# sipposip/pr-disagg-radar-gan

Hardware: AMD Instinct MI355X
Metric: cWGAN-GP train samples/sec, 24x16x16 tiles, bs=256 (higher is better)
Workload: dtype f32; 1 GPU; ndomain=16, 24h, bs=256 fp32, 1 critic step + 1 gen step (BASELINE configs[1]); batch_per_gpu=256, global_batch=256, n_critic=1, parallelism=dp1, world=1, rccl_ranks_seen=1, weights=random init (RandomNormal 0.02 / glorot_uniform), dropout 0.25 active

## Files before the change

### include/rdgan.h

```cpp
#ifndef RDGAN_H
#define RDGAN_H
#include <stdint.h>
#ifdef __cplusplus
extern "C" {
#endif

typedef struct rdgan_handle rdgan_handle;

#define RDGAN_LATENT_DIM 100
#define RDGAN_NHOURS 24
#define RDGAN_LOSS_SLOTS 8

int rdgan_create(rdgan_handle** out, int ndomain, int n_cond_channels, int max_batch);
void rdgan_destroy(rdgan_handle* h);
const char* rdgan_last_error(const rdgan_handle* h);
long rdgan_gen_param_count(const rdgan_handle* h);
long rdgan_critic_param_count(const rdgan_handle* h);
long rdgan_workspace_bytes(const rdgan_handle* h);

int rdgan_gen_forward(rdgan_handle* h, const float* gen_params, const float* z, const float* cond,
                      float* out, int B, void* stream);

int rdgan_check_numerics(rdgan_handle* h, void* stream);

// ... 132 lines not shown
                               int Cin, int Cout, int Do, int Ho, int Wo, int stride, int pad_d, int pad_h,
                               int pad_w, void* stream);
int rdgan_op_fastd_wgrad(const float* src, const float* dy, float* dU, int B, int D, int H, int W, int Cin, int Cout,
                         int g, int bf16, void* stream);
int rdgan_op_g9_wgrad(const float* dl, const float* h3, float* dW, int B, int nd, int bf16, int kernel, void* stream);
int rdgan_op_upconv_slab16(const float* x, const float* w, const float* bias, float* y, float* rinv, float* dbg, int B, void* stream);
int rdgan_op_upconv_slab_t16(const float* x, const float* w, const float* bias, float* y, float* rinv, float* dbg, int B, int H, int W,
                             void* stream);
int rdgan_op_upconv2_slab16(const float* x, const float* w, const float* bias, float* y, float* rinv, int B, void* stream);
int rdgan_op_upconv_wgrad_slab16(const float* x, const float* dy, float* dWc, int B, void* stream);
int rdgan_op_d2_fwd_slab16(const float* x, const float* w, const float* bias, float* y, int B, uint64_t seed, void* stream);
int rdgan_op_d2_wgrad_slab16(const float* x, const float* dy, float* dW, int B, void* stream);
int rdgan_op_d2_wgrad_slab_t16(const float* x, const float* dy, float* dW, int B, int OH, int OW, void* stream);
int rdgan_op_d3_wgrad_slab16(const float* x, const float* dy, float* dW, int B, void* stream);
int rdgan_op_d2_dgrad_slab16(const float* gy, const float* w, const float* aux, float* gx, int B, int use_drop, void* stream);
int rdgan_op_d2_dgrad_slab_t16(const float* gy, const float* w, const float* aux, float* gx, int B, int OH, int OW, int use_drop,
                               void* stream);
int rdgan_op_pixelnorm_lrelu(const float* y, float* h, float* rinv, long npix, int C, void* stream);
int rdgan_op_pixelnorm_lrelu_bwd(const float* gh, const float* h, const float* rinv, float* dy,
                                 long npix, int C, void* stream);
int rdgan_debug_activation(rdgan_handle* h, int which, float* out, long n, void* stream);
int rdgan_debug_d1_input_grad(rdgan_handle* h, const float* critic_params, const float* u1, int B, int with_norm,
                              float* g0_out, float* cin_hat_out, float* gp_out, void* stream);
int rdgan_op_rng(uint64_t seed, uint32_t stream_id, float* mask_out, float* uniform_out, long n,
                 void* stream);

#ifdef __cplusplus
}
#endif
#endif
```

### pr_disagg_radar_gan_amd/_lib.py

```python
import ctypes
import os

_HERE = os.path.dirname(os.path.abspath(__file__))
LIB_PATH = os.path.join(_HERE, "librdgan_hip.so")

c_f32p = ctypes.c_void_p
c_stream = ctypes.c_void_p

class LaunchStat(ctypes.Structure):
    _fields_ = [("plan", ctypes.c_int), ("kind", ctypes.c_int), ("batch", ctypes.c_int), ("launches", ctypes.c_int),
                ("gflop", ctypes.c_double), ("ms", ctypes.c_double), ("name", ctypes.c_char * 48), ("kernel", ctypes.c_char * 48)]


SIGNATURES = {
    "rdgan_create": (ctypes.c_int, [ctypes.POINTER(ctypes.c_void_p), ctypes.c_int, ctypes.c_int, ctypes.c_int]),
    "rdgan_destroy": (None, [ctypes.c_void_p]),
    "rdgan_last_error": (ctypes.c_char_p, [ctypes.c_void_p]),
    "rdgan_gen_param_count": (ctypes.c_long, [ctypes.c_void_p]),
    "rdgan_critic_param_count": (ctypes.c_long, [ctypes.c_void_p]),
    "rdgan_workspace_bytes": (ctypes.c_long, [ctypes.c_void_p]),
    "rdgan_gen_forward": (ctypes.c_int, [ctypes.c_void_p, c_f32p, c_f32p, c_f32p, c_f32p, ctypes.c_int, c_stream]),
    "rdgan_check_numerics": (ctypes.c_int, [ctypes.c_void_p, c_stream]),
    "rdgan_critic_forward": (ctypes.c_int, [ctypes.c_void_p, c_f32p, c_f32p, c_f32p, c_f32p, ctypes.c_int,
                                            ctypes.c_uint64, c_stream]),
# ... 73 lines not shown
    "rdgan_op_conv3d": (ctypes.c_int, [c_f32p, c_f32p, c_f32p, c_f32p] + [ctypes.c_int] * 14 + [c_stream]),
    "rdgan_op_conv3d_bf16": (ctypes.c_int, [c_f32p, c_f32p, c_f32p, c_f32p] + [ctypes.c_int] * 14 + [c_stream]),
    "rdgan_op_conv3d_dgrad": (ctypes.c_int, [c_f32p, c_f32p, c_f32p] + [ctypes.c_int] * 13 + [c_stream]),
    "rdgan_op_conv3d_wgrad_bf16": (ctypes.c_int, [c_f32p, c_f32p, c_f32p] + [ctypes.c_int] * 13 + [c_stream]),
    "rdgan_op_conv3d_dgrad_bf16": (ctypes.c_int, [c_f32p, c_f32p, c_f32p] + [ctypes.c_int] * 13 + [c_stream]),
    "rdgan_op_conv3d_wgrad": (ctypes.c_int, [c_f32p, c_f32p, c_f32p] + [ctypes.c_int] * 14 + [c_stream]),
    "rdgan_op_fastd_wgrad": (ctypes.c_int, [c_f32p, c_f32p, c_f32p] + [ctypes.c_int] * 8 + [c_stream]),
    "rdgan_op_g9_wgrad": (ctypes.c_int, [c_f32p, c_f32p, c_f32p] + [ctypes.c_int] * 4 + [c_stream]),
    "rdgan_op_upconv_slab16": (ctypes.c_int, [c_f32p] * 6 + [ctypes.c_int, c_stream]),
    "rdgan_op_upconv_slab_t16": (ctypes.c_int, [c_f32p] * 6 + [ctypes.c_int] * 3 + [c_stream]),
    "rdgan_op_upconv2_slab16": (ctypes.c_int, [c_f32p] * 5 + [ctypes.c_int, c_stream]),
    "rdgan_op_upconv_wgrad_slab16": (ctypes.c_int, [c_f32p] * 3 + [ctypes.c_int, c_stream]),
    "rdgan_op_d2_fwd_slab16": (ctypes.c_int, [c_f32p] * 4 + [ctypes.c_int, ctypes.c_uint64, c_stream]),
    "rdgan_op_d3_wgrad_slab16": (ctypes.c_int, [c_f32p] * 3 + [ctypes.c_int, c_stream]),
    "rdgan_op_d2_wgrad_slab16": (ctypes.c_int, [c_f32p] * 3 + [ctypes.c_int, c_stream]),
    "rdgan_op_d2_wgrad_slab_t16": (ctypes.c_int, [c_f32p] * 3 + [ctypes.c_int] * 3 + [c_stream]),
    "rdgan_op_d2_dgrad_slab16": (ctypes.c_int, [c_f32p] * 4 + [ctypes.c_int, ctypes.c_int, c_stream]),
    "rdgan_op_d2_dgrad_slab_t16": (ctypes.c_int, [c_f32p] * 4 + [ctypes.c_int] * 4 + [c_stream]),
    "rdgan_op_pixelnorm_lrelu": (ctypes.c_int, [c_f32p, c_f32p, c_f32p, ctypes.c_long, ctypes.c_int, c_stream]),
    "rdgan_op_pixelnorm_lrelu_bwd": (ctypes.c_int, [c_f32p, c_f32p, c_f32p, c_f32p, ctypes.c_long, ctypes.c_int, c_stream]),
    "rdgan_debug_activation": (ctypes.c_int, [ctypes.c_void_p, ctypes.c_int, c_f32p, ctypes.c_long, c_stream]),
    "rdgan_debug_d1_input_grad": (ctypes.c_int, [ctypes.c_void_p, c_f32p, c_f32p, ctypes.c_int, ctypes.c_int, c_f32p, c_f32p, c_f32p,
                                                 c_stream]),
    "rdgan_op_rng": (ctypes.c_int, [ctypes.c_uint64, ctypes.c_uint32, c_f32p, c_f32p, ctypes.c_long, c_stream]),
}

TAG_GCONV_FWD, TAG_GCONV_DGRAD, TAG_GCONV_WGRAD, TAG_CRITIC_GEMM, TAG_ELEMENTWISE, TAG_GCONV3_FWD = range(6)

_lib = None


class RdganError(RuntimeError):
    pass


class NumericsError(RdganError, ArithmeticError):
    """tf.debugging.check_numerics behind the generator's softmax (reference T:349-350) fired: NaN/Inf in the output."""


def load():
    global _lib
    if _lib is not None:
        return _lib
    if not os.path.exists(LIB_PATH):
        raise RdganError(
            f"{LIB_PATH} is missing: build it with `python -m pr_disagg_radar_gan_amd.build` "
# ... 19 lines not shown
```

### pr_disagg_radar_gan_amd/csrc/rdgan_api.hip

```cpp
#include <hip/hip_runtime.h>
#include <stdio.h>
#include <string.h>
#include <math.h>
#include <string>
#include <vector>
#include <algorithm>
#include <unordered_set>

#include "../../include/rdgan.h"
#include "rdgan_plan.h"
#include "rdgan_hostplan.h"
#include "rdgan_rng.h"
#include "rdgan_gemm.hip.h"
#include "rdgan_gemm_ws.hip.h"
#include "rdgan_gemm_ws16.hip.h"
#include "rdgan_gemm_f16.hip.h"
#include "rdgan_upconv16.hip.h"
#include "rdgan_upconv16b.hip.h"
#include "rdgan_upconv16t.hip.h"
#include "rdgan_elem.hip.h"
#include "rdgan_data.hip.h"
#include "rdgan_edge.hip.h"
#include "rdgan_d2slab16.hip.h"
#include "rdgan_d2fwd16.hip.h"
#include "rdgan_upwgrad16.hip.h"
#include "rdgan_upwgrad16b.hip.h"
#include "rdgan_d2wgrad16.hip.h"
#include "rdgan_d3wgrad16.hip.h"
#include "rdgan_d1fwd16.hip.h"
#include "rdgan_g9bwd16.hip.h"
#include "rdgan_spectral.hip.h"
#include "rdgan_rainfarm.hip.h"
#include "rdgan_crps.hip.h"
#include "rdgan_dist.hip.h"
#include "rdgan_radar.hip.h"
#include "rdgan_field.hip.h"
#include "rdgan_products.hip.h"
static_assert(RDGAN_LOSS_SLOTS == 8, "k_critic_losses / k_gen_loss write slots 0..7");
static bool g9w_mfma_ok(int nd, long npix) { return nd >= 8 && nd <= 128 && (nd & (nd - 1)) == 0 && npix < 0x7FFFFFFFL; }
static size_t g9w_mfma_lds(bool bf16) { return std::max<size_t>((size_t)128 * (bf16 ? 128 : 256) + (1440 + 144) * sizeof(float), 32768); }

#define RD_GP_WEIGHT 10.0f



struct RdLaunchRec { int plan, kind, batch; double flops; char kernel[48]; hipEvent_t e0, e1; };

struct rdgan_handle : RdGeom {
  std::string err;
  std::vector<RdPlan> plans;
  RdPlan* d_plans = nullptr;
  RdRow* d_tab = nullptr;
  char* ws = nullptr;
  size_t ws_bytes = 0;
  float *xcat, *h0, *h1, *r1, *h2, *r2, *h3, *r3, *P9, *fake, *dl, *gh3, *gup3, *dy2, *gup2, *dy1, *gup1, *ga0;
  float *cin, *dh[5], *du[5], *v, *P1, *g0, *gpv;
  float* ubias_part = nullptr;
  float *wpartial, *cpartial, *kpartial;
  size_t wpartial_cap = 0, cpartial_cap = 0, kpartial_cap = 0;
  float *DWT[5], *W1T, *GWT[4], *W9T, *W1P, *dW1P;
  float *fE[4], *fU[4], *fgS, *fdE, *fdU, *fUT;
  void *bU[4], *bUT;
  void *bWF[5], *bWB[5];
  void *bG1F[4], *bG1B, *bW1B;
  void *fWF[5], *fWB[5], *fG1F[4], *fG1B;
  int wgrad_wide = 0;
  int conv_f16 = 1;
  void* bW3I;
// ... 26 lines not shown
  int d2_slab = 1;
  int a16 = 0;
  int g9_direct = 1;
  int fast_fwd = -1;
  int fast_bwd = -1;
  float *GWC[4], *GWD[4], *dWc;
  int collapse = 1;
  int tapgather = 1;
  int ws_ksplit = 1;
  int wave_spec = 1;
  int resident = 1;
  int edge_kernels = 1;
  int sample_offset = 0;
  float* g9b_tmp;
  float* gp_part;
  float* dw6_part;
  int side_on = 1;
  int split3 = 0;
  int dense_slices = 0;
  uint64_t gver_in = 0, cver_in = 0;
  const float* gcache_ptr = nullptr; uint64_t gcache_ver = 0; int gcache_cfg = -1;
  const float* ccache_ptr = nullptr; uint64_t ccache_ver = 0; int ccache_cfg = -1;
  long form_builds[2] = {0, 0};
  int keep_gates = 0;
  void* gate_keep[5] = {nullptr, nullptr, nullptr, nullptr, nullptr};
  int gate_keep_B = 0;
  hipStream_t side = nullptr;
  hipEvent_t ev_fork = nullptr, ev_join = nullptr, ev_cw = nullptr, ev_g[4] = {nullptr, nullptr, nullptr, nullptr};
  int* d_flag;
  int fwd_ahead = -1;
  hipStream_t ahead = nullptr;
  hipEvent_t ev_ahead_fork = nullptr, ev_ahead_done = nullptr;
  float* kpartial_ahead = nullptr;
  int* flag_ahead = nullptr;
  bool ahead_pending = false;
  const float *ahead_gp = nullptr, *ahead_z = nullptr, *ahead_cond = nullptr;
  int ahead_B = 0;
  uint64_t ahead_gver = 0;
  std::unordered_set<const void*> lds_attr_done;
  int prof_launches = 0;
  std::vector<RdLaunchRec> launch_recs;
  size_t launch_used = 0;
  char cur_kernel[48] = {0};
  double flops_acc = 0;
  unsigned prof_mask = 0;
  std::vector<hipEvent_t> ev_start[RDGAN_NUM_TAGS], ev_stop[RDGAN_NUM_TAGS];
// ... 741 lines not shown
          carve(p, 27L * dch[l - 1] * dch[l] / 2 + 8); h->bWF[l] = p;
          carve(p, 27L * dch[l - 1] * dch[l] / 2 + 8); h->bWB[l] = p;
        }
        h->bG1F[0] = nullptr;
        for (int l = 1; l <= 3; ++l) { carve(p, 32L * gch[l - 1] * gch[l] + 8); h->bG1F[l] = p; }
        carve(p, 32L * 256 * 256 + 8); h->bG1B = p;
        h->fWF[0] = h->fWF[1] = h->fWB[0] = h->fWB[1] = h->fG1F[0] = nullptr;
        for (int l = 2; l <= 4; ++l) {
          carve(p, 27L * dch[l - 1] * dch[l] / 2 + 8); h->fWF[l] = p;
          carve(p, 27L * dch[l - 1] * dch[l] / 2 + 8); h->fWB[l] = p;
        }
        for (int l = 1; l <= 3; ++l) { carve(p, 32L * gch[l - 1] * gch[l] + 8); h->fG1F[l] = p; }
        carve(p, 32L * 256 * 256 + 8); h->fG1B = p;
        carve(p, 32L * h->ldp1 + 8); h->bW1B = p;
        carve(p, 64L * 8 * 2 * 64 * 4 + 8); h->bW3I = p;
        carve(p, 64L * 8 * 2 * 64 * 4 + 8); h->bW3T = p;
        carve(p, 4L * 64 * 4 + 8); h->bW9I = p;
        carve(p, (long)RD_UP2_KSTEPS * 4 * 64 * 4 + 8); h->bW2I = p;
        carve(p, (long)RD_D2S_KSTEPS * 2 * 64 * 4 + 8); h->bW2S = p;
        if (nd % 16 == 0) { carve(p, NB * h->dL[1] * 4 + 8); if (pass == 1) h->g1bits = (unsigned char*)p; }
        carve(p, (long)RD_D2F_KSTEPS * 4 * 64 * 4 + 8); h->bW2F = p;
      }
      carve(h->fdU, 48L * 256 * 256); carve(h->fUT, 48L * 256 * 256);
    }
    { float* f = nullptr; carve(f, 64); if (pass == 1) { h->d_flag = (int*)f; h->flag_ahead = (int*)f + 32; } }
    carve(h->g9b_tmp, 64);
    carve(h->ubias_part, 32 * 8 * 64);
    carve(h->gp_part, (size_t)MB * 64);
    carve(h->dw6_part, (size_t)16 * h->F);
    if (pass == 0) {
      h->ws_bytes = off + 256;
      e = hipMalloc((void**)&h->ws, h->ws_bytes);
      if (e != hipSuccess) { (void)hipFree(h->d_plans); delete h; return (int)e; }
      (void)hipMemset(h->ws, 0, h->ws_bytes);
    }
  }
  {
    bool ok = hipStreamCreateWithFlags(&h->side, hipStreamNonBlocking) == hipSuccess;
    hipEvent_t* evs[] = {&h->ev_fork, &h->ev_join, &h->ev_cw, &h->ev_g[1], &h->ev_g[2], &h->ev_g[3]};
    for (hipEvent_t* e2 : evs) ok = ok && hipEventCreateWithFlags(e2, hipEventDisableTiming) == hipSuccess;
    if (!ok) { h->side_on = 0; (void)hipGetLastError(); }
    bool ok2 = hipStreamCreateWithFlags(&h->ahead, hipStreamNonBlocking) == hipSuccess;
    ok2 = ok2 && hipEventCreateWithFlags(&h->ev_ahead_fork, hipEventDisableTiming) == hipSuccess;
    ok2 = ok2 && hipEventCreateWithFlags(&h->ev_ahead_done, hipEventDisableTiming) == hipSuccess;
    if (!ok2) { h->ahead = nullptr; (void)hipGetLastError(); }
  }
// ... 45 lines not shown
    if (value && !a16_geometry_ok(h->nd)) return bad_arg(h, RD_A16_TOO_LARGE);
    h->a16 = value ? 1 : 0; return 0;
  }
  if (!strcmp(name, "g9_direct")) { h->g9_direct = value ? 1 : 0; return 0; }
  if (!strcmp(name, "fast_fwd")) { h->fast_fwd = value < 0 ? -1 : (value ? 1 : 0); return 0; }
  if (!strcmp(name, "fast_bwd")) { h->fast_bwd = value < 0 ? -1 : (value ? 1 : 0); return 0; }
  if (!strcmp(name, "tapgather")) { h->tapgather = value ? 1 : 0; return 0; }
  if (!strcmp(name, "resident")) { h->resident = value ? 1 : 0; return 0; }
  if (!strcmp(name, "upconv_slab")) { h->upconv_slab = value ? 1 : 0; return 0; }
  if (!strcmp(name, "upconv_slab_t")) { h->upconv_slab_t = value ? 1 : 0; return 0; }
  if (!strcmp(name, "upconv2_slab")) { h->upconv2_slab = value ? 1 : 0; return 0; }
  if (!strcmp(name, "g9_fused")) { h->g9_fused = value ? 1 : 0; return 0; }
  if (!strcmp(name, "d1_fwd_sample")) { h->d1_fwd_sample = value ? 1 : 0; return 0; }
  if (!strcmp(name, "g9_bwd_mfma")) { h->g9_bwd_mfma = value ? 1 : 0; return 0; }
  if (!strcmp(name, "dense16")) { h->dense16 = value ? 1 : 0; return 0; }
  if (!strcmp(name, "dense_skinny")) { h->dense_skinny = value ? 1 : 0; return 0; }
  if (!strcmp(name, "wgrad_boxes")) { h->wgrad_boxes = value ? 1 : 0; return 0; }
  if (!strcmp(name, "border_boxes")) { h->border_boxes = value < 0 ? 0 : (value > 2 ? 2 : value); return 0; }
  if (!strcmp(name, "d3_wgrad_slab")) { h->d3_wgrad_slab = value ? 1 : 0; return 0; }
  if (!strcmp(name, "d2_wgrad_slab")) { h->d2_wgrad_slab = value ? 1 : 0; return 0; }
  if (!strcmp(name, "upwgrad_slab")) { h->upwgrad_slab = value ? 1 : 0; return 0; }
  if (!strcmp(name, "d1_dgrad_fused")) { h->d1_dgrad_fused = value ? 1 : 0; return 0; }
  if (!strcmp(name, "combine_dx_fused")) { h->combine_dx_fused = value ? 1 : 0; return 0; }
  if (!strcmp(name, "d1_wgrad16")) { h->d1_wgrad16 = value ? 1 : 0; return 0; }
  if (!strcmp(name, "wgrad_wide")) { h->wgrad_wide = value ? 1 : 0; return 0; }
  if (!strcmp(name, "conv_f16")) {
    if (value < 0 || value > 2) return bad_arg(h, "conv_f16: 0, 1 or 2 (2: regardless of the launch size)");
    h->conv_f16 = value; h->ccache_ver = 0; h->gcache_ver = 0; return 0;
  }
  if (!strcmp(name, "d2_fwd_slab")) { h->d2_fwd_slab = value ? 1 : 0; h->ccache_ver = 0; return 0; }
  if (!strcmp(name, "d2_gate_bits")) { h->d2_gate_bits = value ? 1 : 0; return 0; }
  if (!strcmp(name, "d2_slab")) { h->d2_slab = value ? 1 : 0; h->ccache_ver = 0; return 0; }
  if (!strcmp(name, "dense_wgrad_slices")) { h->dense_slices = value; return 0; }
  if (!strcmp(name, "keep_gates")) {
    h->keep_gates = value ? 1 : 0;
    h->gate_keep_B = 0;
    for (int l = 1; l <= 4 && h->keep_gates; ++l)
      if (!h->gate_keep[l]) RD_CHECK(h, hipMalloc(&h->gate_keep[l], (size_t)h->MB * h->dL[l] * h->dch[l] * sizeof(float)));
    return 0;
  }
  if (!strcmp(name, "split3")) { h->split3 = value ? 1 : 0; return 0; }
  if (!strcmp(name, "side_stream")) { h->side_on = (value && h->side) ? 1 : 0; return 0; }
  if (!strcmp(name, "gen_fwd_ahead")) { h->fwd_ahead = value < 0 ? -1 : (value ? 1 : 0); return 0; }
  if (!strcmp(name, "edge_kernels")) { h->edge_kernels = value < 0 ? 0 : (value > 2 ? 2 : value); return 0; }
  if (!strcmp(name, "sample_offset")) { if (value < 0) return bad_arg(h, "set_option: sample_offset < 0"); h->sample_offset = value; return 0; }
  if (!strcmp(name, "ws_ksplit")) { h->ws_ksplit = value < 0 ? 0 : (value > 8 ? 8 : value); return 0; }
// ... 157 lines not shown
static int critic_dgrad_plan(const rdgan_handle* h, int l, int n) {
  return critic_box_plan(h, PL_D2B + l - 2, PL_D2BX + l - 2, (long)n * h->dL[l - 1]);
}

static bool box_span_ok(const RdPlan& p, int B) {
  long minL = p.ph[0].L;
  for (int i = 1; i < p.nphases; ++i) minL = std::min<long>(minL, p.ph[i].L);
  return std::min<long>(B, 256 / minL + 2) * std::max(p.src_sample, p.dst_sample) * 4 < 0x7FFFFFF0L;
}
static int gen_box_plan(const rdgan_handle* h, int one, int box, int B) {
  if (!h->border_boxes || !h->plans[box].boxes || !box_span_ok(h->plans[box], B)) return one;
  if (h->border_boxes >= 2) return box;
  if (plan_flops(h->plans[box], 1) > 0.7 * plan_flops(h->plans[one], 1)) return one;
  return plan_tiles(h->plans[one], B, 128) * (h->plans[one].N / 128 > 0 ? h->plans[one].N / 128 : 1) >= 1024 ? box : one;
}

static int dense_skinny_ks(const rdgan_handle* h) { return (h->n_in + 127) / 128 * 8; }
static bool dense_skinny_on(const rdgan_handle* h) {
  return h->a16 && h->dense16 && h->dense_skinny && h->MB <= 128 && h->bW0 && h->xcat16 && h->n_nodes % 32 == 0 && h->KP0 % 64 == 0;
}
static bool g9_fused_on(const rdgan_handle* h) { return h->g9_fused && h->tapgather && upconv_slab_on(h, 3); }
static bool g9_fused_t_on(const rdgan_handle* h) { return h->g9_fused && h->tapgather && upconv_slab_t_on(h, 3); }

static int gen_forward_impl(rdgan_handle* h, const float* gp, const float* z, const float* cond, float* out, int B,
                            hipStream_t st, hipStream_t ws, bool keep_h3 = true) {
  const int nd = h->nd;
  const bool a16 = h->a16 != 0;
  RD_TRY(a16_check(h));
  const int gcfg = (h->collapse ? 1 : 0) | (fast_fwd_on(h) ? 2 : 0) | (a16 ? 4 : 0) | (h->upconv_slab ? 8 : 0) | (h->upconv2_slab ? 16 : 0) |
                   (h->g9_fused && h->tapgather ? 32 : 0) | (h->dense16 ? 64 : 0) | (h->upconv_slab_t ? 128 : 0) | (h->dense_skinny ? 256 : 0);
  const bool forms_cached = h->gver_in != 0 && gp == h->gcache_ptr && h->gver_in == h->gcache_ver && gcfg == h->gcache_cfg;
  if (!forms_cached) {
  h->form_builds[0]++;
  h->gcache_ptr = nullptr; h->gcache_ver = 0; h->gcache_cfg = -1;
  RD_TRY(launch_transpose(h, gp + h->goff[8], h->W9T, 1, 27, 64, 32, ws));
  if (dense_skinny_on(h)) {
    const long nimg = (long)(h->n_nodes / 32) * dense_skinny_ks(h) * 16;
    hipLaunchKernelGGL(k_dense_wimg, dim3((unsigned)((nimg + 255) / 256)), dim3(256), 0, ws, gp + h->goff[0], (unsigned short*)h->bW0,
                       h->n_in, h->n_nodes, dense_skinny_ks(h));
  } else
  if (a16 && h->dense16 && h->dense16_ok && h->bW0)
    hipLaunchKernelGGL(k_dense_w16, dim3((h->n_nodes + 31) / 32, (h->KP0 + 31) / 32), dim3(256), 0, ws, gp + h->goff[0],
                       (unsigned short*)h->bW0, h->n_in, h->n_nodes, h->KP0);
  if (g9_fused_on(h) || g9_fused_t_on(h)) hipLaunchKernelGGL(k_g9_wimg, dim3(1), dim3(256), 0, ws, gp + h->goff[8], (unsigned short*)h->bW9I);
  for (int l = 1; l <= 3; ++l) {
    const float* Wl = gp + h->goff[2 * l];
    const long cc = (long)h->gch[l - 1] * h->gch[l];
    if (gen_block_fast(h, l, fast_fwd_on(h))) {
      RdWeightMap wm;
      fastd_weight_map(wm);
      ProfScope ps(h, RDGAN_TAG_ELEMENTWISE, ws);
      hipLaunchKernelGGL(k_weight_transform, dim3(ew_blocks(48L * cc / 4)), dim3(256), 0, ws, Wl, h->fU[l], (int)cc, 48, wm);
      if (a16) RD_TRY(launch_weights_to_bf16_t(h, h->fU[l], h->bU[l], 48, h->gch[l - 1], h->gch[l], ws));
    } else if (h->collapse) {
      hipLaunchKernelGGL(k_collapse_weights, dim3(ew_blocks(16L * cc)), dim3(256), 0, ws, Wl, h->GWC[l], (int)cc);
      if (upconv_slab_on(h, l)) launch_upconv_wimg(h->GWC[l], h->bW3I, ws);
      else if (upconv_slab_t_on(h, l)) launch_upconv_wimg_t(h->GWC[l], h->bW3T, ws);
      else if (upconv2_slab_on(h, l)) launch_upconv2_wimg(h->GWC[l], h->bW2I, ws);
      else if (a16) {
        RD_TRY(launch_weights_to_bf16_t(h, h->GWC[l], h->bG1F[l], 64, h->gch[l - 1], h->gch[l], ws, h->conv_f16 ? h->fG1F[l] : nullptr));
      }
    }
    if (ws != st) RD_CHECK(h, hipEventRecord(h->ev_g[l], ws));
  }
  RD_CHECK(h, hipGetLastError());
  h->gcache_ptr = gp; h->gcache_ver = h->gver_in; h->gcache_cfg = gcfg;
  }
  {
    ProfScope ps(h, RDGAN_TAG_ELEMENTWISE, st);
    const bool d16 = a16 && h->dense16 && h->dense16_ok && h->xcat16 && !dense_skinny_on(h);
    hipLaunchKernelGGL(k_concat, dim3(ew_blocks((long)B * h->n_in)), dim3(256), 0, st, z, cond, h->xcat, B,
                       RDGAN_LATENT_DIM, nd * nd * h->nc, h->d_flag,
                       d16 ? (unsigned short*)h->xcat16 : (unsigned short*)nullptr, h->KP0);
  }
  if (dense_skinny_on(h)) {
    if (ws != st && !forms_cached) RD_CHECK(h, hipStreamWaitEvent(st, h->ev_g[1], 0));
    const int RB = (B + 31) / 32, KS = dense_skinny_ks(h);
    ProfScope ps(h, -1, st);
    LaunchScope ls(h, PL_GDENSE16, RD_KIND_CONV, B, 3.0 * plan_flops(h->plans[PL_GDENSE16], B), st);
    RD_KNAME(h, "k_dense16_skinny<bf16>");
    h->flops_acc += 3.0 * plan_flops(h->plans[PL_GDENSE16], B);
    hipLaunchKernelGGL(k_concat16f, dim3((unsigned)(((long)KS * RB * 64 + 255) / 256)), dim3(256), 0, st, z, cond, (unsigned short*)h->xcat16, B,
                       RDGAN_LATENT_DIM, nd * nd * h->nc, KS, RB);
    const dim3 dg((unsigned)(h->n_nodes / 32));
    const unsigned short* xi = (const unsigned short*)h->xcat16; const unsigned short* wi = (const unsigned short*)h->bW0;
    const float* bs = gp + h->goff[1];
// ... 679 lines not shown
    const bool mfma = h->edge_kernels && g9w_mfma_ok(nd, npix3) && g9w_partial_floats(g9w_groups(true, B, nd)) <= h->wpartial_cap;
    RD_TRY(launch_g9_wgrad(h, {PL_G9B, 2.0 * npix3 * 64 * 27, RDGAN_TAG_GCONV_WGRAD}, mfma, a16, h->dl, h->h3, h->wpartial, h->wpartial_cap,
                           grad + h->goff[8], B, nd, st));
  } else {
    {
      ProfScope ps(h, RDGAN_TAG_ELEMENTWISE, st);
      hipLaunchKernelGGL(k_dl_im2col, dim3(ew_blocks(npix3 * 8)), dim3(256), 0, st, h->dl, h->P9, B, RDGAN_NHOURS, nd, nd);
    }
    RD_TRY(launch_wgrad(h, h->plans[PL_G9B], h->d_plans + PL_G9B, B, h->P9, h->h3, grad + h->goff[8], h->wpartial,
                        h->wpartial_cap, st, RDGAN_TAG_GCONV_WGRAD));
    RD_TRY(launch_conv(h, h->plans[PL_G9B], h->d_plans + PL_G9B, B, h->P9, gp + h->goff[8], 64, h->gh3,
                       epi_make(RD_EPI_PLAIN), st, RDGAN_TAG_GCONV_DGRAD));
  }
  {
    hipStream_t cs = side_fork(h, st);
    RD_TRY(launch_colsum(h, h->dl, npix3 / 64, 64, h->g9b_tmp, cs));
    RD_TRY(launch_colsum(h, h->g9b_tmp, 64, 1, grad + h->goff[9], cs));
  }
  float* hs[4] = {h->h0, h->h1, h->h2, h->h3};
  float* rs[4] = {nullptr, h->r1, h->r2, h->r3};
  float* dys[4] = {nullptr, h->dy1, h->dy2, h->gh3};
  float* gups[4] = {nullptr, h->gup1, h->gup2, h->gup3};
  const int col = h->collapse;
  const float* dE_in = nullptr;
  if (col) {
    RdSliceMap map;
    collapsed_dgrad_slice_map(map.src);
    for (int l = 1; l <= 3; ++l) {
      if (gen_block_fast(h, l, fast_bwd_on(h))) continue;
      if (gen_block_fast(h, l, fast_fwd_on(h)))
        hipLaunchKernelGGL(k_collapse_weights, dim3(ew_blocks(16L * h->gch[l - 1] * h->gch[l])), dim3(256), 0, st,
                           gp + h->goff[2 * l], h->GWC[l], h->gch[l - 1] * h->gch[l]);
      if (a16) continue;
      hipLaunchKernelGGL(k_transpose_map, dim3((h->gch[l] + 31) / 32, (h->gch[l - 1] + 31) / 32, 64), dim3(256), 0, st,
                         h->GWC[l], h->GWD[l], h->gch[l - 1], h->gch[l], map);
    }
  }
  for (int l = 3; l >= 1; --l) {
    const bool fast = gen_block_fast(h, l, fast_bwd_on(h));
    if (l == 3 && g9_direct) {
      ProfScope ps(h, RDGAN_TAG_ELEMENTWISE, st);
      if (a16 && !fast && h->g9_bwd_mfma && (nd * nd) % 32 == 0) {
        const int PP = nd <= 16 ? 4 : 1;
        const size_t lds9 = (size_t)(2 * PP + 2) * (nd + 2) * (nd + 2) * sizeof(float);
        const int nunits = B * (RDGAN_NHOURS / 2 / PP);
        RD_TRY(ensure_lds(h, (const void*)k_g9_bwd_mfma16, lds9));
        hipLaunchKernelGGL(k_g9_bwd_mfma16, dim3((unsigned)std::min(nunits, PP > 1 ? 768 : 1536)), dim3(256), lds9, st, h->dl, gp + h->goff[8],
                           (const rd_bf16_t*)hs[3], rs[3], (rd_bf16_t*)dys[3], nunits, RDGAN_NHOURS, nd, nd, PP);
// ... 47 lines not shown
          RD_TRY(launch_wgrad16(h, h->plans[pl], h->d_plans + pl, B, wsrc[g], wdy[g], h->fdU, h->wpartial, h->wpartial_cap, st,
                                RDGAN_TAG_GCONV_WGRAD));
        } else
        RD_TRY(launch_wgrad(h, h->plans[pl], h->d_plans + pl, B, wsrc[g], wdy[g], h->fdU, h->wpartial, h->wpartial_cap, st,
                            RDGAN_TAG_GCONV_WGRAD));
      }
      hipLaunchKernelGGL(k_weight_transform_adj, dim3(ew_blocks(27L * cc / 4)), dim3(256), 0, st, h->fdU, grad + h->goff[2 * l],
                         (int)cc, 48, wm);
      RD_TRY(launch_colsum(h, dys[l], (long)B * h->gpix[l], h->gch[l], grad + h->goff[2 * l + 1], side_fork(h, st), a16));
      const int pbs = PL_F1BS + l - 1, pbe = PL_F1BE + l - 1;
      RdEpi eb = epi_make(RD_EPI_PLAIN);
      eb.out16 = a16;
      if (a16) {
        RdSliceMap map;
        fastd_dgrad_slice_map(map.src);
        {
          ProfScope ps(h, RDGAN_TAG_ELEMENTWISE, st);
          hipLaunchKernelGGL(k_blocks_to_bf16, dim3((unsigned)std::min<long>((cc / 8 + 255) / 256, 64), 48), dim3(256), 0, st,
                             h->fU[l], (unsigned short*)h->bUT, cc, map);
        }
        RD_TRY(launch_conv16(h, h->plans[pbs], h->d_plans + pbs, B, h->fgS, h->bUT, gups[l], eb, st, RDGAN_TAG_GCONV_DGRAD));
        RD_TRY(launch_conv16(h, h->plans[pbe], h->d_plans + pbe, B, dys[l], h->bUT, h->fdE, eb, st, RDGAN_TAG_GCONV_DGRAD));
      } else {
        {
          RdSliceMap map;
          fastd_dgrad_slice_map(map.src);
          hipLaunchKernelGGL(k_transpose_map, dim3((h->gch[l] + 31) / 32, (h->gch[l - 1] + 31) / 32, 48), dim3(256), 0, st, h->fU[l],
                             h->fUT, h->gch[l - 1], h->gch[l], map);
        }
        RD_TRY(launch_conv(h, h->plans[pbs], h->d_plans + pbs, B, h->fgS, h->fUT, h->gch[l - 1], gups[l], eb, st,
                           RDGAN_TAG_GCONV_DGRAD));
        RD_TRY(launch_conv(h, h->plans[pbe], h->d_plans + pbe, B, dys[l], h->fUT, h->gch[l - 1], h->fdE, eb, st,
                           RDGAN_TAG_GCONV_DGRAD));
      }
      if (!a16 && h->combine_dx_fused && l >= 2) dE_in = h->fdE;
      else {
        ProfScope ps(h, RDGAN_TAG_ELEMENTWISE, st);
        const dim3 cg(ew_blocks((long)B * D * P / 4));
        if (a16) hipLaunchKernelGGL(k_combine_dx<rd_bf16_t>, cg, dim3(256), 0, st, (rd_bf16_t*)gups[l], (const rd_bf16_t*)h->fdE, B, D, P);
        else hipLaunchKernelGGL(k_combine_dx<float>, cg, dim3(256), 0, st, gups[l], (const float*)h->fdE, B, D, P);
      }
    } else if (col) {
      int plf = PL_G1FC + l - 1, plb = gen_box_plan(h, PL_G1BC + l - 1, PL_G1BCX + l - 1, B);
      const int plfx = PL_G1FCX + l - 1;
      const bool wbox = h->wgrad_boxes && h->border_boxes && h->wave_spec && wgrad_box_ok(h->plans[plfx]) &&
                        (h->border_boxes >= 2 || plan_flops(h->plans[plfx], 1) < 0.8 * plan_flops(h->plans[plf], 1));
      bool bias_done = false;
      if (a16 && l == 3 && h->upwgrad_slab && h->nd == 16) {
        RD_TRY(launch_upconv_wgrad_slab(h, {plf, plan_flops(h->plans[plf], B), RDGAN_TAG_GCONV_WGRAD}, hs[l - 1], dys[l], h->wpartial,
                                        h->wpartial_cap, h->dWc, h->ubias_part, grad + h->goff[2 * l + 1], B, st));
        bias_done = true;
      } else if (a16 && l == 2 && h->upwgrad_slab && h->nd == 16) {
        RD_TRY(launch_upconv2_wgrad_slab(h, {plf, plan_flops(h->plans[plf], B), RDGAN_TAG_GCONV_WGRAD}, hs[l - 1], dys[l], h->wpartial,
                                         h->wpartial_cap, h->dWc, h->ubias_part, grad + h->goff[2 * l + 1], B, st));
        bias_done = true;
// ... 27 lines not shown
      int plf = PL_G1F + l - 1, plb = PL_G1B + l - 1;
      RD_TRY(launch_wgrad(h, h->plans[plf], h->d_plans + plf, B, hs[l - 1], dys[l], grad + h->goff[2 * l], h->wpartial,
                          h->wpartial_cap, st, RDGAN_TAG_GCONV_WGRAD));
      RD_TRY(launch_colsum(h, dys[l], (long)B * h->gpix[l], h->gch[l], grad + h->goff[2 * l + 1], side_fork(h, st)));
      RD_TRY(launch_conv(h, h->plans[plb], h->d_plans + plb, B, dys[l], h->GWT[l], h->gch[l - 1], gups[l],
                         epi_make(RD_EPI_PLAIN), st, RDGAN_TAG_GCONV_DGRAD));
    }
  }
  {
    ProfScope ps(h, RDGAN_TAG_ELEMENTWISE, st);
    const dim3 lg(ew_blocks((long)B * h->gpix[0] * 64));
    if (col && a16)
      hipLaunchKernelGGL(k_lrelu_bwd<rd_bf16_t>, lg, dim3(256), 0, st, (const rd_bf16_t*)h->gup1, (const rd_bf16_t*)h->h0, h->ga0,
                         (long)B * h->gpix[0] * 64);
    else if (col)
      hipLaunchKernelGGL(k_lrelu_bwd<float>, lg, dim3(256), 0, st, (const float*)h->gup1, (const float*)h->h0, h->ga0,
                         (long)B * h->gpix[0] * 64);
    else
      hipLaunchKernelGGL(k_pool_lrelu_bwd, lg, dim3(256), 0, st, h->gup1, h->h0,
                         h->ga0, (long)B * h->gpix[0], h->gdim[0][0], h->gdim[0][1], h->gdim[0][2], 256);
  }
  RD_TRY(launch_wgrad(h, h->plans[PL_GDENSE], h->d_plans + PL_GDENSE, B, h->xcat, h->ga0, grad + h->goff[0], h->wpartial,
                      h->wpartial_cap, st, RDGAN_TAG_GCONV_WGRAD));
  RD_TRY(launch_colsum(h, h->ga0, B, h->n_nodes, grad + h->goff[1], side_fork(h, st)));
  RD_TRY(side_join(h, st, h->ev_join));
  {
    ProfScope ps(h, RDGAN_TAG_ELEMENTWISE, st);
    hipLaunchKernelGGL(k_gen_loss, dim3(1), dim3(256), 0, st, h->v, grad + h->n_gen, B, h->d_flag);
  }
  RD_CHECK(h, hipGetLastError());
  return 0;
}

extern "C" int rdgan_adam(float* params, const float* grad, float* v, long n, int t, float lr, float beta2, float eps,
                          float grad_scale, void* stream) {
  if (!params || !grad || !v || n < 1 || t < 1) return -2;
  float lr_t = lr * sqrtf(1.0f - powf(beta2, (float)t));
  hipLaunchKernelGGL(k_adam, dim3(ew_blocks(n / 4 + 1)), dim3(256), 0, (hipStream_t)stream, params, grad, v, n, lr_t, beta2,
                     eps, grad_scale);
  return (int)hipGetLastError();
}

struct TmpPlan {
  RdPlan host; RdPlan* dev = nullptr; RdRow* tab = nullptr;
  int upload() {
    std::vector<RdRow> t;
    if (!plan_build_tables(host, t)) return -2;
    hipError_t e = hipMalloc((void**)&tab, sizeof(RdRow) * t.size());
// ... 357 lines not shown
  RD_TRY(launch_pn_bwd(nullptr, gh, hh, rinv, dy, npix, C, 0, 0, 0, 0, (hipStream_t)stream));
  return (int)hipStreamSynchronize((hipStream_t)stream);
}

extern "C" int rdgan_debug_d1_input_grad(rdgan_handle* h, const float* critic_params, const float* u1, int B, int with_norm,
                                         float* g0_out, float* cin_hat_out, float* gp_out, void* stream) {
  if (!h || !critic_params || !u1 || !g0_out) return bad_arg(h, "debug_d1_input_grad: null pointer");
  if (with_norm && (!cin_hat_out || !gp_out)) return bad_arg(h, "debug_d1_input_grad: with_norm needs cin_hat_out and gp_out");
  if (B < 1 || B > h->MB) return bad_arg(h, "debug_d1_input_grad: B outside [1, max_batch]");
  if (h->a16) return bad_arg(h, "debug_d1_input_grad: fp32 storage only");
  hipStream_t st = (hipStream_t)stream;
  RD_TRY(ahead_drain(h, st));
  RD_TRY(prep_critic_weights(h, critic_params, st));
  if (with_norm) {
    RD_TRY(critic_penalty_input(h, critic_params, u1, B, h->cin, st));
    RD_CHECK(h, hipMemcpyAsync(cin_hat_out, h->cin, sizeof(float) * B * h->dL[0] * h->CP, hipMemcpyDeviceToDevice, st));
    RD_CHECK(h, hipMemcpyAsync(gp_out, h->gpv, sizeof(float) * B, hipMemcpyDeviceToDevice, st));
  } else
    RD_TRY(critic_input_grad(h, critic_params, u1, B, st));
  RD_CHECK(h, hipMemcpyAsync(g0_out, h->g0, sizeof(float) * B * h->dL[0], hipMemcpyDeviceToDevice, st));
  return 0;
}

__global__ void k_bytes_to_f32(const unsigned char* in, float* out, long n) {
  for (long i = blockIdx.x * (long)blockDim.x + threadIdx.x; i < n; i += (long)gridDim.x * blockDim.x) out[i] = (float)in[i];
}
extern "C" int rdgan_debug_activation(rdgan_handle* h, int which, float* out, long n, void* stream) {
  if (h) RD_TRY(ahead_drain(h, (hipStream_t)stream));
  if (h && out && which == 8 && n >= 1) {
    if (!h->g1bits || n > (long)h->NB * h->dL[1] * 16) return bad_arg(h, "debug_activation: no gate bytes");
    hipLaunchKernelGGL(k_bytes_to_f32, dim3(ew_blocks(n)), dim3(256), 0, (hipStream_t)stream, h->g1bits, out, n);
    RD_CHECK(h, hipGetLastError());
    return 0;
  }
  if (!h || !out || which < 0 || which > 7 || n < 1) return bad_arg(h, "debug_activation: bad argument");
  const float* src; long cap;
  if (which < 4) {
    float* hs[4] = {h->h0, h->h1, h->h2, h->h3};
    src = hs[which]; cap = (long)h->MB * h->gpix[which] * h->gch[which];
  } else {
    const int l = which - 3;
    src = h->dh[l]; cap = (long)h->NB * h->dL[l] * h->dch[l];
  }
  if (n > cap) return bad_arg(h, "debug_activation: n exceeds the tensor");
  hipStream_t st = (hipStream_t)stream;
  auto copy = [&](const void* from, long first, long cnt) -> int {
// ... 553 lines not shown
```

### pr_disagg_radar_gan_amd/engine.py

```python
import ctypes
import itertools

import numpy as np
import torch

from . import _lib
from . import weights as W

LOSS_SLOTS = 8

_versions = itertools.count(1)


def new_version():
    return next(_versions)


def require_gpu():
    if not torch.cuda.is_available():
        raise _lib.RdganError("no MI355X/ROCm device visible: the cWGAN-GP hot path runs only on the HIP "
                              "library (there is deliberately no CPU fallback)")


def _ptr(t):
# ... 165 lines not shown
    def profile(self, tag_mask):
        _lib.check(self.lib.rdgan_profile(self._h, int(tag_mask)), self._h, "rdgan_profile")

    def debug_activation(self, which, shape):
        out = torch.empty(tuple(shape), dtype=torch.float32, device=self.device)
        _lib.check(self.lib.rdgan_debug_activation(self._h, int(which), _ptr(out), out.numel(), self._stream()), self._h,
                   "rdgan_debug_activation")
        return out

    def debug_d1_input_grad(self, critic_params, u1, with_norm=False):
        B, nd = u1.shape[0], self.ndomain
        self._check_batch(B, self.max_batch)
        _chk_tensor(critic_params, (self.n_critic,), "critic_params")
        _chk_tensor(u1, (B, u1.shape[1], 64), "u1")
        g0 = torch.empty((B, W.NHOURS, nd, nd), dtype=torch.float32, device=self.device)
        cin_hat = torch.empty((B, W.NHOURS * nd * nd, 1 + self.n_cond_channels), dtype=torch.float32, device=self.device) if with_norm else None
        gp = torch.empty((B,), dtype=torch.float32, device=self.device) if with_norm else None
        _lib.check(self.lib.rdgan_debug_d1_input_grad(self._h, _ptr(critic_params), _ptr(u1), B, int(bool(with_norm)), _ptr(g0),
                                                      ctypes.c_void_p(cin_hat.data_ptr() if with_norm else 0),
                                                      ctypes.c_void_p(gp.data_ptr() if with_norm else 0), self._stream()),
                   self._h, "rdgan_debug_d1_input_grad")
        return (g0, cin_hat, gp) if with_norm else g0

    def flop_count(self, reset=False):
        f = ctypes.c_double()
        _lib.check(self.lib.rdgan_flop_count(self._h, ctypes.byref(f), int(bool(reset))), self._h, "rdgan_flop_count")
        return f.value

    def profile_launches(self, on):
        _lib.check(self.lib.rdgan_profile_launches(self._h, int(bool(on))), self._h, "rdgan_profile_launches")

    def launch_table(self):
        buf = (_lib.LaunchStat * 256)()
        n = ctypes.c_int()
        _lib.check(self.lib.rdgan_launch_table(self._h, buf, 256, ctypes.byref(n)), self._h, "rdgan_launch_table")
        kinds = {0: "gemm", 1: "wgrad", 2: "edge"}
        return [dict(name=r.name.decode(), kernel=r.kernel.decode(), kind=kinds.get(r.kind, "?"), batch=r.batch,
                     launches=r.launches, gflop=r.gflop, ms=r.ms) for r in buf[:n.value]]

    def profile_read(self, tag):
        ms, n = ctypes.c_double(), ctypes.c_long()
        _lib.check(self.lib.rdgan_profile_read(self._h, int(tag), ctypes.byref(ms), ctypes.byref(n)), self._h,
                   "rdgan_profile_read")
        return ms.value, n.value
```

Baseline: 24060 samples/s.

## Prebuild generator backward weight forms on side stream during forward form build

When the generator weight forms are built for a given parameter version, the transposed dgrad slice forms for the three upconv blocks are now also built on the side stream and kept in per-layer buffers. The backward pass then reuses them instead of rebuilding and transposing them on the main stream. A second change runs the dense bias column sum on the main stream after the join instead of forking it. This adds per-layer buffers and debug APIs, and the gain depends on the forward form build overlapping other work.

```diff
diff --git a/include/rdgan.h b/include/rdgan.h
--- a/include/rdgan.h
+++ b/include/rdgan.h
@@ -178,6 +178,9 @@
 int rdgan_debug_activation(rdgan_handle* h, int which, float* out, long n, void* stream);
 int rdgan_debug_d1_input_grad(rdgan_handle* h, const float* critic_params, const float* u1, int B, int with_norm,
                               float* g0_out, float* cin_hat_out, float* gp_out, void* stream);
+long rdgan_debug_weight_form_size(const rdgan_handle* h, int which);
+int rdgan_debug_weight_form(rdgan_handle* h, const float* params, int which, int rebuild, float* out, long n, void* stream);
+int rdgan_bform_builds(const rdgan_handle* h, long* builds);
 int rdgan_op_rng(uint64_t seed, uint32_t stream_id, float* mask_out, float* uniform_out, long n,
                  void* stream);
 
diff --git a/pr_disagg_radar_gan_amd/_lib.py b/pr_disagg_radar_gan_amd/_lib.py
--- a/pr_disagg_radar_gan_amd/_lib.py
+++ b/pr_disagg_radar_gan_amd/_lib.py
@@ -119,6 +119,9 @@
     "rdgan_debug_activation": (ctypes.c_int, [ctypes.c_void_p, ctypes.c_int, c_f32p, ctypes.c_long, c_stream]),
     "rdgan_debug_d1_input_grad": (ctypes.c_int, [ctypes.c_void_p, c_f32p, c_f32p, ctypes.c_int, ctypes.c_int, c_f32p, c_f32p, c_f32p,
                                                  c_stream]),
+    "rdgan_debug_weight_form_size": (ctypes.c_long, [ctypes.c_void_p, ctypes.c_int]),
+    "rdgan_debug_weight_form": (ctypes.c_int, [ctypes.c_void_p, c_f32p, ctypes.c_int, ctypes.c_int, c_f32p, ctypes.c_long, c_stream]),
+    "rdgan_bform_builds": (ctypes.c_int, [ctypes.c_void_p, ctypes.POINTER(ctypes.c_long)]),
     "rdgan_op_rng": (ctypes.c_int, [ctypes.c_uint64, ctypes.c_uint32, c_f32p, c_f32p, ctypes.c_long, c_stream]),
 }
 
diff --git a/pr_disagg_radar_gan_amd/csrc/rdgan_api.hip b/pr_disagg_radar_gan_amd/csrc/rdgan_api.hip
--- a/pr_disagg_radar_gan_amd/csrc/rdgan_api.hip
+++ b/pr_disagg_radar_gan_amd/csrc/rdgan_api.hip
@@ -44,6 +44,7 @@
 
 
 
+enum { RD_LEAN_BFORMS = 1, RD_LEAN_DENSE = 2 };
 struct RdLaunchRec { int plan, kind, batch; double flops; char kernel[48]; hipEvent_t e0, e1; };
 
 struct rdgan_handle : RdGeom {
@@ -116,6 +117,10 @@
   const float* gcache_ptr = nullptr; uint64_t gcache_ver = 0; int gcache_cfg = -1;
   const float* ccache_ptr = nullptr; uint64_t ccache_ver = 0; int ccache_cfg = -1;
   long form_builds[2] = {0, 0};
+  int lean_joins = -1, lean_items = 3;
+  float* fUTl[4] = {nullptr, nullptr, nullptr, nullptr};
+  bool bforms_built = false;
+  long bform_builds = 0;
   int keep_gates = 0;
   void* gate_keep[5] = {nullptr, nullptr, nullptr, nullptr, nullptr};
   int gate_keep_B = 0;
@@ -903,6 +908,7 @@
         carve(p, (long)RD_D2F_KSTEPS * 4 * 64 * 4 + 8); h->bW2F = p;
       }
       carve(h->fdU, 48L * 256 * 256); carve(h->fUT, 48L * 256 * 256);
+      for (int l = 1; l <= 3; ++l) carve(h->fUTl[l], 48L * gch[l - 1] * gch[l]);
     }
     { float* f = nullptr; carve(f, 64); if (pass == 1) { h->d_flag = (int*)f; h->flag_ahead = (int*)f + 32; } }
     carve(h->g9b_tmp, 64);
@@ -994,6 +1000,8 @@
   if (!strcmp(name, "upwgrad_slab")) { h->upwgrad_slab = value ? 1 : 0; return 0; }
   if (!strcmp(name, "d1_dgrad_fused")) { h->d1_dgrad_fused = value ? 1 : 0; return 0; }
   if (!strcmp(name, "combine_dx_fused")) { h->combine_dx_fused = value ? 1 : 0; return 0; }
+  if (!strcmp(name, "lean_joins")) { h->lean_joins = value < 0 ? -1 : (value ? 1 : 0); return 0; }
+  if (!strcmp(name, "lean_joins_items")) { h->lean_items = value & 3; return 0; }
   if (!strcmp(name, "d1_wgrad16")) { h->d1_wgrad16 = value ? 1 : 0; return 0; }
   if (!strcmp(name, "wgrad_wide")) { h->wgrad_wide = value ? 1 : 0; return 0; }
   if (!strcmp(name, "conv_f16")) {
@@ -1197,18 +1205,32 @@
 static bool g9_fused_on(const rdgan_handle* h) { return h->g9_fused && h->tapgather && upconv_slab_on(h, 3); }
 static bool g9_fused_t_on(const rdgan_handle* h) { return h->g9_fused && h->tapgather && upconv_slab_t_on(h, 3); }
 
+static bool lean_on(const rdgan_handle* h, int item) { return (h->lean_joins < 0 ? !h->a16 : h->lean_joins) && (h->lean_items & item); }
+static bool lean_bforms_on(const rdgan_handle* h) {
+  return lean_on(h, RD_LEAN_BFORMS) && !h->a16 && h->collapse && fast_fwd_on(h) == fast_bwd_on(h);
+}
+static int gen_form_cfg(const rdgan_handle* h) {
+  return (h->collapse ? 1 : 0) | (fast_fwd_on(h) ? 2 : 0) | (h->a16 ? 4 : 0) | (h->upconv_slab ? 8 : 0) | (h->upconv2_slab ? 16 : 0) |
+         (h->g9_fused && h->tapgather ? 32 : 0) | (h->dense16 ? 64 : 0) | (h->upconv_slab_t ? 128 : 0) | (h->dense_skinny ? 256 : 0) |
+         (lean_bforms_on(h) ? 512 : 0);
+}
+static bool lean_bforms_ready(const rdgan_handle* h, const float* gp) {
+  return h->bforms_built && lean_bforms_on(h) && gp == h->gcache_ptr && h->gver_in == h->gcache_ver && gen_form_cfg(h) == h->gcache_cfg;
+}
+
 static int gen_forward_impl(rdgan_handle* h, const float* gp, const float* z, const float* cond, float* out, int B,
                             hipStream_t st, hipStream_t ws, bool keep_h3 = true) {
   const int nd = h->nd;
   const bool a16 = h->a16 != 0;
   RD_TRY(a16_check(h));
-  const int gcfg = (h->collapse ? 1 : 0) | (fast_fwd_on(h) ? 2 : 0) | (a16 ? 4 : 0) | (h->upconv_slab ? 8 : 0) | (h->upconv2_slab ? 16 : 0) |
-                   (h->g9_fused && h->tapgather ? 32 : 0) | (h->dense16 ? 64 : 0) | (h->upconv_slab_t ? 128 : 0) | (h->dense_skinny ? 256 : 0);
+  const int gcfg = gen_form_cfg(h);
+  const bool bforms = lean_bforms_on(h);
   const bool forms_cached = h->gver_in != 0 && gp == h->gcache_ptr && h->gver_in == h->gcache_ver && gcfg == h->gcache_cfg;
   if (!forms_cached) {
   h->form_builds[0]++;
   h->gcache_ptr = nullptr; h->gcache_ver = 0; h->gcache_cfg = -1;
-  RD_TRY(launch_transpose(h, gp + h->goff[8], h->W9T, 1, 27, 64, 32, ws));
+  h->bforms_built = false;
+  if (!bforms) RD_TRY(launch_transpose(h, gp + h->goff[8], h->W9T, 1, 27, 64, 32, ws));
   if (dense_skinny_on(h)) {
     const long nimg = (long)(h->n_nodes / 32) * dense_skinny_ks(h) * 16;
     hipLaunchKernelGGL(k_dense_wimg, dim3((unsigned)((nimg + 255) / 256)), dim3(256), 0, ws, gp + h->goff[0], (unsigned short*)h->bW0,
@@ -1221,6 +1243,7 @@
   for (int l = 1; l <= 3; ++l) {
     const float* Wl = gp + h->goff[2 * l];
     const long cc = (long)h->gch[l - 1] * h->gch[l];
+    if (bforms && l == 3) RD_TRY(launch_transpose(h, gp + h->goff[8], h->W9T, 1, 27, 64, 32, ws));
     if (gen_block_fast(h, l, fast_fwd_on(h))) {
       RdWeightMap wm;
       fastd_weight_map(wm);
@@ -1237,6 +1260,21 @@
       }
     }
     if (ws != st) RD_CHECK(h, hipEventRecord(h->ev_g[l], ws));
+  }
+  if (bforms) {
+    for (int l = 1; l <= 3; ++l) {
+      RdSliceMap map;
+      const dim3 tg((h->gch[l] + 31) / 32, (h->gch[l - 1] + 31) / 32, 1);
+      if (gen_block_fast(h, l, fast_bwd_on(h))) {
+        fastd_dgrad_slice_map(map.src);
+        hipLaunchKernelGGL(k_transpose_map, dim3(tg.x, tg.y, 48), dim3(256), 0, ws, h->fU[l], h->fUTl[l], h->gch[l - 1], h->gch[l], map);
+      } else {
+        collapsed_dgrad_slice_map(map.src);
+        hipLaunchKernelGGL(k_transpose_map, dim3(tg.x, tg.y, 64), dim3(256), 0, ws, h->GWC[l], h->GWD[l], h->gch[l - 1], h->gch[l], map);
+      }
+    }
+    h->bform_builds++;
+    h->bforms_built = true;
   }
   RD_CHECK(h, hipGetLastError());
   h->gcache_ptr = gp; h->gcache_ver = h->gver_in; h->gcache_cfg = gcfg;
@@ -1962,8 +2000,9 @@
   float* dys[4] = {nullptr, h->dy1, h->dy2, h->gh3};
   float* gups[4] = {nullptr, h->gup1, h->gup2, h->gup3};
   const int col = h->collapse;
+  const bool bready = lean_bforms_ready(h, gp);
   const float* dE_in = nullptr;
-  if (col) {
+  if (col && !bready) {
     RdSliceMap map;
     collapsed_dgrad_slice_map(map.src);
     for (int l = 1; l <= 3; ++l) {
@@ -2057,15 +2096,16 @@
         RD_TRY(launch_conv16(h, h->plans[pbs], h->d_plans + pbs, B, h->fgS, h->bUT, gups[l], eb, st, RDGAN_TAG_GCONV_DGRAD));
         RD_TRY(launch_conv16(h, h->plans[pbe], h->d_plans + pbe, B, dys[l], h->bUT, h->fdE, eb, st, RDGAN_TAG_GCONV_DGRAD));
       } else {
-        {
+        const float* fUT = bready ? h->fUTl[l] : h->fUT;
+        if (!bready) {
           RdSliceMap map;
           fastd_dgrad_slice_map(map.src);
           hipLaunchKernelGGL(k_transpose_map, dim3((h->gch[l] + 31) / 32, (h->gch[l - 1] + 31) / 32, 48), dim3(256), 0, st, h->fU[l],
                              h->fUT, h->gch[l - 1], h->gch[l], map);
         }
-        RD_TRY(launch_conv(h, h->plans[pbs], h->d_plans + pbs, B, h->fgS, h->fUT, h->gch[l - 1], gups[l], eb, st,
+        RD_TRY(launch_conv(h, h->plans[pbs], h->d_plans + pbs, B, h->fgS, fUT, h->gch[l - 1], gups[l], eb, st,
                            RDGAN_TAG_GCONV_DGRAD));
-        RD_TRY(launch_conv(h, h->plans[pbe], h->d_plans + pbe, B, dys[l], h->fUT, h->gch[l - 1], h->fdE, eb, st,
+        RD_TRY(launch_conv(h, h->plans[pbe], h->d_plans + pbe, B, dys[l], fUT, h->gch[l - 1], h->fdE, eb, st,
                            RDGAN_TAG_GCONV_DGRAD));
       }
       if (!a16 && h->combine_dx_fused && l >= 2) dE_in = h->fdE;
@@ -2139,8 +2179,13 @@
   }
   RD_TRY(launch_wgrad(h, h->plans[PL_GDENSE], h->d_plans + PL_GDENSE, B, h->xcat, h->ga0, grad + h->goff[0], h->wpartial,
                       h->wpartial_cap, st, RDGAN_TAG_GCONV_WGRAD));
+  if (lean_on(h, RD_LEAN_DENSE)) {
+    RD_TRY(side_join(h, st, h->ev_join));
+    RD_TRY(launch_colsum(h, h->ga0, B, h->n_nodes, grad + h->goff[1], st));
+  } else {
   RD_TRY(launch_colsum(h, h->ga0, B, h->n_nodes, grad + h->goff[1], side_fork(h, st)));
   RD_TRY(side_join(h, st, h->ev_join));
+  }
   {
     ProfScope ps(h, RDGAN_TAG_ELEMENTWISE, st);
     hipLaunchKernelGGL(k_gen_loss, dim3(1), dim3(256), 0, st, h->v, grad + h->n_gen, B, h->d_flag);
@@ -2544,6 +2589,70 @@
   return 0;
 }
 
+static long weight_form_size(const rdgan_handle* h, int which) {
+  if (which >= 0 && which <= 2) return 27L * h->dch[which + 1] * h->dch[which + 2];
+  if (which == 3) return 64L * h->ldp1;
+  if (which >= 4 && which <= 6) {
+    const int l = which - 3;
+    return (gen_block_fast(h, l, fast_bwd_on(h)) ? 48L : 64L) * h->gch[l - 1] * h->gch[l];
+  }
+  return -1;
+}
+extern "C" long rdgan_debug_weight_form_size(const rdgan_handle* h, int which) { return h ? weight_form_size(h, which) : -1; }
+extern "C" int rdgan_bform_builds(const rdgan_handle* h, long* builds) {
+  if (!h || !builds) return -2;
+  *builds = h->bform_builds;
+  return 0;
+}
+extern "C" int rdgan_debug_weight_form(rdgan_handle* h, const float* params, int which, int rebuild, float* out, long n, void* stream) {
+  if (!h || !params || !out) return bad_arg(h, "debug_weight_form: null pointer");
+  if (h->a16 || !h->collapse || fast_fwd_on(h) != fast_bwd_on(h)) return bad_arg(h, "debug_weight_form: fp32 storage, default forms only");
+  const long sz = weight_form_size(h, which);
+  if (sz < 0 || n != sz || sz > 64L * 256 * 256 || (size_t)sz > h->wpartial_cap) return bad_arg(h, "debug_weight_form: bad form index or size");
+  float* tmp = h->dWc;
+  float* built = h->wpartial;
+  hipStream_t st = (hipStream_t)stream;
+  RD_TRY(ahead_drain(h, st));
+  const float* src = nullptr;
+  if (which <= 3) {
+    const int l = which + 2;
+    if (!rebuild) {
+      if (params != h->ccache_ptr) return bad_arg(h, "debug_weight_form: the critic forms belong to another slab");
+      src = which == 3 ? h->W1T : h->DWT[l];
+    } else {
+      if (which == 3) RD_TRY(launch_transpose(h, params + h->doff[0], built, 1, 27 * h->Cin, 64, h->ldp1, st));
+      else RD_TRY(launch_transpose(h, params + h->doff[2 * (l - 1)], built, 27, h->dch[l - 1], h->dch[l], h->dch[l - 1], st));
+      src = built;
+    }
+  } else {
+    const int l = which - 3;
+    const bool fast = gen_block_fast(h, l, fast_bwd_on(h));
+    if (!rebuild) {
+      if (!lean_bforms_ready(h, params)) return bad_arg(h, "debug_weight_form: no backward forms built ahead for this slab and version");
+      src = fast ? h->fUTl[l] : h->GWD[l];
+    } else {
+      const long cc = (long)h->gch[l - 1] * h->gch[l];
+      RdSliceMap map;
+      const dim3 tg((h->gch[l] + 31) / 32, (h->gch[l - 1] + 31) / 32, fast ? 48 : 64);
+      if (fast) {
+        RdWeightMap wm;
+        fastd_weight_map(wm);
+        fastd_dgrad_slice_map(map.src);
+        hipLaunchKernelGGL(k_weight_transform, dim3(ew_blocks(48L * cc / 4)), dim3(256), 0, st, params + h->goff[2 * l], tmp, (int)cc, 48, wm);
+        hipLaunchKernelGGL(k_transpose_map, tg, dim3(256), 0, st, tmp, built, h->gch[l - 1], h->gch[l], map);
+      } else {
+        collapsed_dgrad_slice_map(map.src);
+        hipLaunchKernelGGL(k_collapse_weights, dim3(ew_blocks(16L * cc)), dim3(256), 0, st, params + h->goff[2 * l], tmp, (int)cc);
+        hipLaunchKernelGGL(k_transpose_map, tg, dim3(256), 0, st, tmp, built, h->gch[l - 1], h->gch[l], map);
+      }
+      RD_CHECK(h, hipGetLastError());
+      src = built;
+    }
+  }
+  RD_CHECK(h, hipMemcpyAsync(out, src, sizeof(float) * n, hipMemcpyDeviceToDevice, st));
+  return 0;
+}
+
 __global__ void k_bytes_to_f32(const unsigned char* in, float* out, long n) {
   for (long i = blockIdx.x * (long)blockDim.x + threadIdx.x; i < n; i += (long)gridDim.x * blockDim.x) out[i] = (float)in[i];
 }
diff --git a/pr_disagg_radar_gan_amd/engine.py b/pr_disagg_radar_gan_amd/engine.py
--- a/pr_disagg_radar_gan_amd/engine.py
+++ b/pr_disagg_radar_gan_amd/engine.py
@@ -211,6 +211,20 @@
                    self._h, "rdgan_debug_d1_input_grad")
         return (g0, cin_hat, gp) if with_norm else g0
 
+    def debug_weight_form(self, params, which, rebuild=False):
+        n = int(self.lib.rdgan_debug_weight_form_size(self._h, int(which)))
+        if n < 0:
+            raise ValueError(f"no weight form {which}")
+        out = torch.empty(n, dtype=torch.float32, device=self.device)
+        _lib.check(self.lib.rdgan_debug_weight_form(self._h, _ptr(params), int(which), int(bool(rebuild)), _ptr(out), n,
+                                                    self._stream()), self._h, "rdgan_debug_weight_form")
+        return out
+
+    def bform_builds(self):
+        n = ctypes.c_long()
+        _lib.check(self.lib.rdgan_bform_builds(self._h, ctypes.byref(n)), self._h, "rdgan_bform_builds")
+        return n.value
+
     def flop_count(self, reset=False):
         f = ctypes.c_double()
         _lib.check(self.lib.rdgan_flop_count(self._h, ctypes.byref(f), int(bool(reset))), self._h, "rdgan_flop_count")
```

New measurement: 24120 samples/s, median of 6. About the same (+0.2%).
